# StractOrg/stract

Hardware: AMD Instinct MI355X
Metric: HyperBall traversed edges/sec (GTEPS) (higher is better)
Workload: dtype u8

## Files before the change

stract_amd/_lib.py:

```python
import ctypes
import os

os.environ.setdefault("OMP_WAIT_POLICY", "passive")

import numpy as np

_HERE = os.path.dirname(os.path.abspath(__file__))
LIB_PATH = os.environ.get("HB_LIB_PATH") or os.path.join(_HERE, "lib", "libhyperball.so")
LIB_EXP_PATH = os.environ.get("HB_LIB_PATH") or os.path.join(_HERE, "lib", "libhyperball_exp.so")

HB_OK = 0
HB_ERR_INVALID, HB_ERR_NO_DEVICE, HB_ERR_HIP, HB_ERR_NOMEM, HB_ERR_RCCL, HB_ERR_LIMIT, HB_ERR_IO = -1, -2, -3, -4, -5, -6, -7
HB_STORE_F64, HB_STORE_U64 = 0, 1
HB_COLL_U8, HB_COLL_U32, HB_COLL_U64, HB_COLL_F64 = 0, 1, 2, 3
HB_COLL_MAX, HB_COLL_SUM = 0, 1
HB_SKIPPED_REL_MASK = 0x6FED00

HB_FLAG_NO_FRONTIER = 0x01
HB_FLAG_NO_REORDER = 0x02
HB_FLAG_UNFUSED = 0x04
HB_FLAG_PASS_STATS = 0x08
HB_FLAG_NO_XCD_MAP = 0x20
HB_FLAG_NO_RCCL = 0x40
HB_FLAG_RCCL_SELF = 0x80
HB_FLAG_NO_SPARSE = 0x100
HB_FLAG_DEST_PARTITION = 0x200
HB_FLAG_HOST_INGEST = 0x400
HB_FLAG_HOST_PLAN = 0x800
HB_FLAG_CHANGED_ONLY = 0x1000
HB_FLAG_REFERENCE_TAIL = 0x2000
HB_FLAG_NO_INIT_PASS = 0x4000
HB_FLAG_ALL_RELS = 0x8000
HB_SAMPLE_MAX_LEVELS = 16

HB_X_TILE_EPILOGUE = 0x100
HB_X_SEED_3LAUNCH = 0x800
HB_X_NO_EDGE_OVERLAP = 0x1000
HB_X_BITMAP_SLOTWISE = 0x2000
HB_X_NO_STAGED_RESULTS = 0x4000
HB_X_SNAPSHOT_EVERY_PASS = 0x8000
HB_X_SHORT_FINAL_LIST = 0x10000
HB_X_ONE_SNAPSHOT = 0x20000
HB_X_NO_TAIL_PIPELINE = 0x100000
HB_X_TAIL_KERNEL = 0x200000
HB_X_TAIL_KERNEL_ANY = 0x400000
HB_X_FULL_INIT = 0x800000
HB_X_WIRE_64B = 0x1000000
HB_X_SCATTER_TRANSPOSE = 0x2000000
HB_X_SWEEP_ROUNDS = 0x4000000
HB_X_GENERIC_LEVEL1 = 0x8000000
HB_X_PROBE_NO_SIZE = 0x10000000

U128 = np.dtype([("lo", "<u8"), ("hi", "<u8")])
EDGE = np.dtype([("from", U128), ("to", U128), ("rel_flags", "<u8")])
assert U128.itemsize == 16 and EDGE.itemsize == 40


class HbOptions(ctypes.Structure):
    _fields_ = [
        ("struct_size", ctypes.c_uint32),
        ("device", ctypes.c_int32),
        ("flags", ctypes.c_uint32),
        ("chunk", ctypes.c_uint32),
        ("max_passes", ctypes.c_uint32),
        ("rank", ctypes.c_int32),
        ("world_size", ctypes.c_int32),
        ("rccl_id", ctypes.c_uint8 * 128),
        ("tune", ctypes.c_uint32 * 8),
    ]


class HbStats(ctypes.Structure):
    _fields_ = [
        ("n", ctypes.c_uint64),
        ("m_input", ctypes.c_uint64),
        ("m_unique", ctypes.c_uint64),
        ("m_eff", ctypes.c_uint64),
        ("passes", ctypes.c_uint64),
        ("results", ctypes.c_uint64),
        ("ms_ingest", ctypes.c_double),
        ("ms_plan", ctypes.c_double),
        ("ms_h2d", ctypes.c_double),
        ("ms_loop", ctypes.c_double),
        ("ms_loop_gpu", ctypes.c_double),
        ("ms_collective", ctypes.c_double),
        ("ms_d2h", ctypes.c_double),
        ("work_rows", ctypes.c_uint64),
        ("virtual_rows", ctypes.c_uint64),
        ("device_bytes", ctypes.c_uint64),
        ("virtual_edges", ctypes.c_uint64),
        ("levels", ctypes.c_uint64),
        ("level1_edges", ctypes.c_uint64),
        ("level1_rows", ctypes.c_uint64),
        ("direct_edges", ctypes.c_uint64),
        ("rows_with_in_edges", ctypes.c_uint64),
# ... 971 lines not shown
```

stract_amd/csrc/hb_api.hip:

```cpp
#include "hb_guard_alloc.h"
#include "hb_pool.h"
#include <hip/hip_runtime.h>
#include <rccl/rccl.h>

#include <algorithm>
#include <cmath>
#include <cstdio>
#include <cstring>
#include <string>
#include <thread>
#include <vector>

#include "hb_internal.h"
#include "hb_experiments.h"
#include "hb_kernels.hip.h"
#include "hb_walk.hip.h"
#include "hb_sample.hip.h"
#include "hb_bfs.hip.h"
#include "hb_betweenness.hip.h"
#include "hb_similarity.hip.h"
#include "hb_nearest_seed.hip.h"
#ifdef HB_EXPERIMENTS
#include "hb_experiments.hip.h"
#endif
// ... 61 lines not shown
};
}

struct GraphDeviceState {
    uint64_t *d_row_ptr = nullptr;
    uint32_t *d_src = nullptr;
    uint16_t *d_src_jp = nullptr;
    bool level0_all_real = false;
    uint32_t *d_virt_rows = nullptr;
    uint16_t *d_self_jp = nullptr;
    uint4 *d_regs[2] = {nullptr, nullptr};
    uint4 *d_part = nullptr;
    uint32_t *d_bits[2] = {nullptr, nullptr};
    uint32_t *d_kdirty = nullptr;
    double *d_ksum = nullptr, *d_kerr = nullptr;
    uint64_t *d_size = nullptr;
    uint64_t *d_idlow = nullptr;
    uint32_t *d_dev_of = nullptr;
    uint32_t *d_sid_of = nullptr;
    uint32_t *d_outdeg = nullptr;
    unsigned long long *d_counters = nullptr;
    double *d_raw = nullptr, *d_bias = nullptr;
    uint8_t *d_lc = nullptr;
    uint64_t *d_out_ptr = nullptr;
    uint32_t *d_out_rows = nullptr;
    uint32_t *d_touch = nullptr;
    uint32_t *d_seeds = nullptr, *d_heavy = nullptr;
    unsigned int *d_sparse_counts = nullptr;
    bool sparse_ok = false;
    uint4 *d_pack = nullptr;
    uint32_t *d_wpop = nullptr;
    uint64_t *d_wprefix = nullptr;
    uint32_t *d_lbits = nullptr, *d_lbits_all = nullptr, *d_ubits = nullptr;
    bool ubits_valid = false;
    unsigned long long *d_rank_cnt = nullptr;
    uint32_t *d_tl_changed[2] = {nullptr, nullptr}, *d_tl_vchanged[2] = {nullptr, nullptr}, *d_tl_dirty[2] = {nullptr, nullptr};
    uint32_t *d_tl_work = nullptr, *d_tl_count = nullptr;
    bool tl_valid = false;
    uint64_t *d_tail_ptr = nullptr;
    uint32_t *d_tail_to = nullptr;
    uint64_t tail_count = 0;
    std::vector<uint64_t> tail_keys;
    std::vector<TailDoc> tail_open;
    bool tail_dirty = false;
    TailIndex *tail_index = nullptr;
    uint32_t *d_bloom = nullptr;
    unsigned long long *d_bloom_ones = nullptr;
    uint32_t *d_list = nullptr;
    double *d_out = nullptr;
    double *h_out = nullptr;
    uint64_t h_out_len = 0;
    uint64_t out_len = 0;
    uint32_t *d_cid_of = nullptr;
    std::vector<uint64_t> h_in_bits;
    struct ResultSync {
        bool on = false;
        bool valid = false;
        uint64_t changed_since = 0;
        uint32_t stages = 0;
        double *d_sent = nullptr;
        uint32_t *d_sid = nullptr;
        double *d_val = nullptr;
        unsigned long long *d_count = nullptr;
        unsigned long long *d_kept = nullptr;
        uint32_t *h_sid = nullptr;
        double *h_val = nullptr;
        unsigned long long *h_count = nullptr;
        uint64_t cap = 0;
    } rs;
    struct SampleState {
        DevPtr<uint16_t> d_hist;
        uint32_t levels = 0;
        DevPtr<unsigned long long> d_cnt;
        DevPtr<uint32_t> d_srcs;
        DevPtr<uint32_t> d_rows;
        DevPtr<double> d_w;
        std::vector<uint32_t> cand;
        bool cand_valid = false;
    } smp;
    struct DistanceState {
        bool ready = false;
        bool valid = false;
        bool extracted = false;
        uint8_t *d_dist = nullptr;
        uint32_t *d_vis = nullptr, *d_front = nullptr, *d_next = nullptr;
        uint32_t *d_heavy = nullptr;
        uint32_t heavy_cap = 0;
        unsigned int *d_heavy_cnt = nullptr;
        unsigned long long *d_cnt = nullptr;
        uint32_t *d_indeg = nullptr;
        bool indeg_valid = false;
        uint8_t *d_by_sid = nullptr;
        uint32_t *d_sel_sid = nullptr;
        uint8_t *d_sel_dist = nullptr;
        uint64_t *d_sel_cnt = nullptr;
        uint64_t words_total = 0;
        uint64_t reached = 0;
    } dst;
    struct BetweennessState {
        bool ready = false;
        bool valid = false;
        uint8_t *d_dist = nullptr;
        unsigned long long *d_sigma = nullptr;
        double *d_delta = nullptr;
        uint8_t *d_reached = nullptr;
        double *d_sum = nullptr;
// ... 1016 lines not shown
        const Plan &p = c->plan;
        double t0 = now_ms();
        if ((rc = ensure_initial_state(c))) return rc;
        if (linked(c) && p.n_pad) {
            HB_COLL(coll_all_gather(c, c->d_ksum + (uint64_t)c->opt.rank * c->slice_rows, c->d_ksum, c->slice_rows, ncclDouble, c->stream));
        }
        const double norm = (double)(p.n ? p.n - 1 : 0);
        unsigned long long *cnt = c->d_counters + (size_t)c->max_passes * hbk::kCounterWords;
        HB_HIP(hipMemsetAsync(cnt, 0, hbk::kCounterWords * sizeof(unsigned long long), c->stream));
        bool shipped = false;
        if (p.n && c->rs.on && c->rs.valid) {
            auto &rs = c->rs;
            HB_HIP(hipMemsetAsync(rs.d_count, 0, sizeof(unsigned long long), c->stream));
            const unsigned blocks = grid_blocks(c, (p.n_pad + 2047) / 2048, 8);
            hipLaunchKernelGGL(hbk::results_sync_kernel, dim3(blocks), dim3(256), 0, c->stream, (const double *)c->d_ksum, rs.d_sent,
                               (const uint32_t *)c->d_cid_of, p.n_pad, norm, 0, c->d_out, rs.d_sid, rs.d_val, (unsigned long long)rs.cap, rs.d_count, cnt);
            HB_HIP(hipGetLastError());
            HB_HIP(hipMemcpyAsync(rs.h_count, rs.d_count, sizeof(unsigned long long), hipMemcpyDeviceToHost, c->stream));
            HB_HIP(hipMemcpyAsync(c->h_counters, cnt, hbk::kCounterWords * sizeof(unsigned long long), hipMemcpyDeviceToHost, c->stream));
            HB_HIP(hipStreamSynchronize(c->stream));
            const uint64_t moved = *rs.h_count;
            if (moved <= rs.cap) {
                if (moved) {
                    HB_HIP(hipMemcpyAsync(rs.h_sid, rs.d_sid, moved * sizeof(uint32_t), hipMemcpyDeviceToHost, c->stream));
                    HB_HIP(hipMemcpyAsync(rs.h_val, rs.d_val, moved * sizeof(double), hipMemcpyDeviceToHost, c->stream));
                    HB_HIP(hipStreamSynchronize(c->stream));
                }
                HB_HIP(hipEventSynchronize(c->rs_copied));
                host_scatter_f64(c->h_out, rs.h_sid, rs.h_val, moved);
            } else {
                HB_HIP(hipStreamWaitEvent(c->stream, c->rs_copied, 0));
                HB_HIP(hipMemcpyAsync(c->h_out, c->d_out, c->out_len * sizeof(double), hipMemcpyDeviceToHost, c->stream));
                HB_HIP(hipStreamSynchronize(c->stream));
            }
            shipped = true;
        }
        if (p.n && !shipped) {
            if (c->rs.on) {
                const unsigned blocks = grid_blocks(c, (p.n_pad + 2047) / 2048, 8);
                hipLaunchKernelGGL(hbk::results_sync_kernel, dim3(blocks), dim3(256), 0, c->stream, (const double *)c->d_ksum, c->rs.d_sent,
                                   (const uint32_t *)c->d_cid_of, p.n_pad, norm, 1, c->d_out, (uint32_t *)nullptr, (double *)nullptr, 0ull, c->rs.d_count, cnt);
            } else {
                unsigned blocks = grid_blocks(c, (p.n + 255) / 256, 8);
                hipLaunchKernelGGL(hbk::finish_kernel, dim3(blocks), dim3(256), 0, c->stream, (const double *)c->d_ksum,
                                   (const uint32_t *)c->d_dev_of, p.n, norm, c->d_out, cnt);
            }
            HB_HIP(hipGetLastError());
            HB_HIP(hipMemcpyAsync(c->h_out, c->d_out, c->out_len * sizeof(double), hipMemcpyDeviceToHost, c->stream));
        }
        if (!shipped) {
            HB_HIP(hipMemcpyAsync(c->h_counters, cnt, hbk::kCounterWords * sizeof(unsigned long long), hipMemcpyDeviceToHost, c->stream));
            HB_HIP(hipStreamSynchronize(c->stream));
        }
        if (std::getenv("HB_TRACE_RESULTS"))
            std::fprintf(stderr, "[hb results] hb_finish: entered at %.3f ms, done at %.3f ms (host clock); %u snapshots, list %llu\n", t0, now_ms(), c->rs.stages,
                         shipped ? (unsigned long long)*c->rs.h_count : 0ull);
        c->stats.pipelined_passes = c->pipelined_passes;
        c->stats.tail_kernel_passes = c->tail_kernel_passes;
        c->stats.result_stages = c->rs.stages;
        c->stats.result_list = shipped ? *c->rs.h_count : 0;
        c->rs.valid = false;
        c->res_count = 0;
        for (int s = 0; s < hbk::kStripes; s++) c->res_count += c->h_counters[4 * s];
        c->stats.ms_d2h = now_ms() - t0;
        c->stats.results = c->res_count;
        c->stats.passes = c->t;
        if ((rc = resolve_pass_times(c))) return rc;
        double g = 0, coll = 0;
        for (auto &ps : c->pstats) { g += ps.ms_gpu; coll += ps.ms_collective; }
        c->stats.ms_loop_gpu = g;
        c->stats.ms_collective = coll;
        c->stats.wire_bytes = c->wire_bytes;
        c->run_open = false;
        c->image = Image::HyperBall;
        return HB_OK;
    });
}

int hb_run(hb_ctx *c, hb_stats *stats)
{
    return guarded(c, [&]() -> int {
        if (!c) return HB_ERR_INVALID;
        int rc = hb_begin(c);
        if (rc) return rc;
        double t0 = now_ms();
        int has = 1;
        const bool trace = std::getenv("HB_TRACE_RESULTS") != nullptr;
        while (has) {
            if (tail_kernel_ready(c)) {
                uint32_t ran = 0;
                if ((rc = tail_kernel_run(c, 64, &ran))) return rc;
                has = c->has_changes ? 1 : 0;
                if (ran) continue;
            }
            if (tail_pipeline_ready(c)) {
                if ((rc = tail_pipeline(c, &has))) return rc;
                continue;
            }
            if ((rc = hb_step(c, &has))) return rc;
            if (trace) std::fprintf(stderr, "[hb results] pass %llu returned at %.3f ms (host clock)\n", (unsigned long long)c->t - 1, now_ms());
        }
        c->stats.ms_loop = now_ms() - t0;
        if ((rc = hb_finish(c))) return rc;
        if (stats) *stats = c->stats;
        return HB_OK;
    });
// ... 147 lines not shown
```

stract_amd/csrc/hb_api_load.inc:

```
bool device_plan(const hb_ctx *c) { return !(c->opt.flags & HB_FLAG_HOST_PLAN); }
bool deferred_times(const hb_ctx *c);

int keep_owned(hb_ctx *c, DeviceCsr *csr)
{
    if (!dest_mode(c)) return HB_OK;
    const uint64_t world = (uint64_t)std::max(c->opt.world_size, 1), rank = (uint64_t)c->opt.rank, n = c->g.ids.size();
    if (c->g.row_ptr.size() == n + 1 && n) keep_owned_rows(&c->g, world, rank);
    if (csr && csr->d_row_ptr) {
        const std::string e = gpu_keep_owned_rows((void *)c->stream, csr, n, world, rank);
        if (!e.empty()) return fail(c, e.find("memory") != std::string::npos ? HB_ERR_NOMEM : HB_ERR_HIP, e);
    }
    return HB_OK;
}

__global__ __launch_bounds__(256) void idlow_kernel(const uint64_t *lo_by_sid, const uint32_t *order, uint64_t n_pad, uint64_t *idlow)
{
    const uint64_t d = (uint64_t)blockIdx.x * 256 + threadIdx.x;
    if (d >= n_pad) return;
    const uint32_t s = order[d];
    idlow[d] = s == kNone ? 0ull : lo_by_sid[s];
}

template <class T>
T *adopt(hb_ctx *c, DevPtr<T> &b, size_t bytes)
// ... 234 lines not shown
            HB_HIP(hipMemcpyAsync(c->d_src, p.src.data(), p.src.size() * sizeof(uint32_t), hipMemcpyHostToDevice, c->stream));
        if (p.n_pad)
            HB_HIP(hipMemcpyAsync(c->d_sid_of, p.order.data(), p.n_pad * sizeof(uint32_t), hipMemcpyHostToDevice, c->stream));
        std::vector<uint32_t> outdeg_dev(p.n_pad, 0);
        c->m_global = 0;
        for (uint64_t d = 0; d < p.n_pad; d++)
            if (p.order[d] != kNone) {
                outdeg_dev[d] = outdeg[p.order[d]];
                c->m_global += outdeg[p.order[d]];
            }
        if (p.n_pad)
            HB_HIP(hipMemcpyAsync(c->d_outdeg, outdeg_dev.data(), p.n_pad * sizeof(uint32_t), hipMemcpyHostToDevice, c->stream));
        if (n) HB_HIP(hipMemcpyAsync(c->d_dev_of, p.dev_of.data(), n * sizeof(uint32_t), hipMemcpyHostToDevice, c->stream));
        HB_HIP(hipStreamSynchronize(c->stream));
    } else {
        uint64_t ends[2] = {0, 0};
        HB_HIP(hipMemcpyAsync(&ends[0], c->d_row_ptr + p.n_pad, sizeof(uint64_t), hipMemcpyDeviceToHost, c->stream));
        HB_HIP(hipMemcpyAsync(&ends[1], c->d_row_ptr + rows_total, sizeof(uint64_t), hipMemcpyDeviceToHost, c->stream));
        HB_HIP(hipStreamSynchronize(c->stream));
        c->stats.virtual_edges = ends[1] - ends[0];
    }
    lap("tables / plan arrays");
    c->out_len = n;
    c->d_cid_of = c->d_sid_of;
    if (c->rs.on && n) {
        DevPtr<uint32_t> d_flags;
        DevPtr<uint64_t> d_cpos;
        DevPtr<unsigned long long> d_words;
        const uint64_t nw = (n + 63) / 64;
        HB_HIP(d_flags.alloc(n + 1));
        HB_HIP(d_cpos.alloc(n + 2));
        HB_HIP(d_words.alloc(nw));
        if ((rc = dev_alloc(c, &c->d_cid_of, p.n_pad))) return rc;
        HB_HIP(hipMemsetAsync(d_flags.get(), 0, (n + 1) * sizeof(uint32_t), c->stream));
        const unsigned blocks = grid_blocks(c, (p.n_pad + 255) / 256, 16);
        hipLaunchKernelGGL(hbk::in_flags_kernel, dim3(blocks), dim3(256), 0, c->stream, (const uint64_t *)c->d_row_ptr, (const uint32_t *)c->d_sid_of, p.n_pad, d_flags.get());
        HB_HIP(hipGetLastError());
        const std::string e = device_prefix((void *)c->stream, d_flags.get(), n, d_cpos.get());
        if (!e.empty()) return fail(c, HB_ERR_HIP, e);
        hipLaunchKernelGGL(hbk::cid_of_kernel, dim3(blocks), dim3(256), 0, c->stream, (const uint64_t *)c->d_row_ptr, (const uint32_t *)c->d_sid_of,
                           (const uint64_t *)d_cpos.get(), p.n_pad, c->d_cid_of);
        HB_HIP(hipGetLastError());
        hipLaunchKernelGGL(hbk::pack_flags_kernel, dim3(grid_blocks(c, (nw + 3) / 4, 16)), dim3(256), 0, c->stream,
                           (const uint32_t *)d_flags.get(), n, d_words.get());
        HB_HIP(hipGetLastError());
        uint64_t n_c = 0;
        c->h_in_bits.assign(nw, 0);
        HB_HIP(hipMemcpyAsync(&n_c, d_cpos.get() + n, sizeof(uint64_t), hipMemcpyDeviceToHost, c->stream));
        HB_HIP(hipMemcpyAsync(c->h_in_bits.data(), d_words.get(), nw * sizeof(uint64_t), hipMemcpyDeviceToHost, c->stream));
        HB_HIP(hipStreamSynchronize(c->stream));
        if (n_c != p.rows_with_in_edges)
            return fail(c, HB_ERR_INVALID, "result image: " + std::to_string(n_c) + " nodes with in-edges counted on the device, the plan says " + std::to_string(p.rows_with_in_edges));
        c->out_len = n_c;
        lap("compact result image (cid per row, host bitmap)");
    }
    if (n) {
        if (!d_lo) {
            uvec<uint64_t> lo(n);
            host_gather_id_lo(c->g.ids.data(), n, lo.data());
            HB_HIP(d_lo.alloc(n));
            HB_HIP(hipMemcpyAsync(d_lo.get(), lo.data(), n * sizeof(uint64_t), hipMemcpyHostToDevice, c->stream));
            HB_HIP(hipStreamSynchronize(c->stream));
        }
        hipLaunchKernelGGL(idlow_kernel, dim3((unsigned)((p.n_pad + 255) / 256)), dim3(256), 0, c->stream, (const uint64_t *)d_lo.get(),
                           (const uint32_t *)c->d_sid_of, p.n_pad, c->d_idlow);
        HB_HIP(hipGetLastError());
        HB_HIP(hipStreamSynchronize(c->stream));
    }
    lap("id_low");
    if (src_len && !(c->opt.flags & HB_FLAG_NO_INIT_PASS)) {
        if ((rc = dev_alloc(c, &c->d_src_jp, src_len + 4))) return rc;
        const unsigned blocks = grid_blocks(c, (src_len + 255) / 256, 16);
        if ((rc = dev_alloc(c, &c->d_self_jp, p.n_pad + 4))) return rc;
        hipLaunchKernelGGL(hbk::self_jp_kernel, dim3(grid_blocks(c, (p.n_pad + 255) / 256, 16)), dim3(256), 0, c->stream,
                           (const uint64_t *)c->d_idlow, (const uint32_t *)c->d_sid_of, p.n_pad, c->d_self_jp);
        HB_HIP(hipGetLastError());
        hipLaunchKernelGGL(hbk::src_jp_kernel, dim3(blocks), dim3(256), 0, c->stream, (const uint32_t *)c->d_src, src_len, (const uint16_t *)c->d_self_jp, p.n_pad,
                           c->d_src_jp);
        HB_HIP(hipGetLastError());
        if ((rc = dev_alloc(c, &c->d_virt_rows, c->bits_words + 4))) return rc;
        unsigned long long *d_l0 = c->d_counters + 8, h_l0 = ~0ull;
        HB_HIP(hipMemsetAsync(d_l0, 0, sizeof(unsigned long long), c->stream));
        const uint64_t l0_lo = p.level_begin.size() > 1 ? p.level_begin[0] : 0, l0_hi = p.level_begin.size() > 1 ? p.level_begin[1] : 0;
        hipLaunchKernelGGL(hbk::virt_rows_kernel, dim3(grid_blocks(c, (rows_total + 255) / 256, 16)), dim3(256), 0, c->stream,
                           (const uint64_t *)c->d_row_ptr, (const uint32_t *)c->d_src, rows_total, p.n_pad, c->d_virt_rows, l0_lo, l0_hi, d_l0);
        HB_HIP(hipGetLastError());
        HB_HIP(hipMemcpyAsync(&h_l0, d_l0, sizeof(h_l0), hipMemcpyDeviceToHost, c->stream));
        HB_HIP(hipStreamSynchronize(c->stream));
        c->level0_all_real = h_l0 == 0;
        HB_HIP(hipStreamSynchronize(c->stream));
    }
    lap("self_jp / src_jp");
    {
        unsigned long long *d_bad = c->d_counters;
        unsigned long long h_bad[4] = {0, 0, 0, 0};
        HB_HIP(hipMemsetAsync(d_bad, 0, sizeof(h_bad), c->stream));
        if (rows_total) {
            const unsigned blocks = grid_blocks(c, (rows_total * 4 + 255) / 256, 16);
            hipLaunchKernelGGL(hbk::validate_plan_kernel, dim3(blocks), dim3(256), 0, c->stream, (const uint64_t *)c->d_row_ptr, (const uint32_t *)c->d_src,
                               rows_total, p.n_pad, src_len, d_bad);
            HB_HIP(hipGetLastError());
        }
        HB_HIP(hipMemcpyAsync(h_bad, d_bad, sizeof(h_bad), hipMemcpyDeviceToHost, c->stream));
        HB_HIP(hipStreamSynchronize(c->stream));
        if (h_bad[0] | h_bad[1] | h_bad[2] | h_bad[3])
            return fail(c, HB_ERR_INVALID, "work layout failed its structural check: " + std::to_string(h_bad[0]) + " bad row pointers, " +
                                               std::to_string(h_bad[1]) + " source ids out of range, " + std::to_string(h_bad[2]) +
// ... 74 lines not shown
```

stract_amd/csrc/hb_api_pass.inc:

```
using PassKernel = void (*)(const hbk::PassParams);
using SweepKernel = void (*)(const hbk::SweepParams);

template <bool REAL, bool FUSED, bool STATS, bool INIT, bool EPI4>
PassKernel dense_by_unroll(int unroll)
{
    if constexpr (!INIT) {
        if (unroll == 1) return hbk::pass_kernel<REAL, FUSED, STATS, 1, INIT, EPI4>;
    }
    if (unroll == 2) return hbk::pass_kernel<REAL, FUSED, STATS, 2, INIT, EPI4>;
    return hbk::pass_kernel<REAL, FUSED, STATS, 4, INIT, EPI4>;
}
template <bool REAL, bool FUSED>
PassKernel dense_kernel_of(bool stats, int unroll, bool init, bool epi4)
{
    if (stats) return dense_by_unroll<REAL, FUSED, true, false, false>(unroll);
    if constexpr (REAL && FUSED) {
        if (epi4) return init ? dense_by_unroll<true, true, false, true, true>(unroll) : dense_by_unroll<true, true, false, false, true>(unroll);
    }
    return init ? dense_by_unroll<REAL, FUSED, false, true, false>(unroll) : dense_by_unroll<REAL, FUSED, false, false, false>(unroll);
}
PassKernel dense_kernel(bool real, bool fused, bool stats, int unroll, bool init, bool epi4)
{
    init = init && unroll != 1;
    if (real && fused) return dense_kernel_of<true, true>(stats, unroll, init, epi4);
// ... 348 lines not shown
        }
        if (!c->exact_counting && bloom_estimate_card(c->bloom_bits, ones) <= c->ref_threshold) c->exact_counting = true;
    }
    c->exact_valid = tracked;
    return HB_OK;
}

int upload_tail_index(hb_ctx *c)
{
    const Plan &p = c->plan;
    std::vector<uint64_t> ptr;
    std::vector<uint32_t> to;
    const std::string e = build_tail_csr(&c->tail_keys, p.n_pad, &ptr, &to);
    if (!e.empty()) return fail(c, HB_ERR_NOMEM, e);
    for (void *old : {(void *)c->d_tail_ptr, (void *)c->d_tail_to}) {
        if (!old) continue;
        for (size_t i = 0; i < c->allocs.size(); i++)
            if (c->allocs[i].p == old) {
                c->stats.device_bytes -= c->allocs[i].bytes;
                (void)hipFree(old);
                c->allocs.erase(c->allocs.begin() + (long)i);
                break;
            }
    }
    c->d_tail_ptr = nullptr;
    c->d_tail_to = nullptr;
    int rc;
    if ((rc = dev_alloc(c, &c->d_tail_ptr, p.n_pad + 1))) return rc;
    if ((rc = dev_alloc(c, &c->d_tail_to, to.size() + 1))) return rc;
    HB_HIP(hipMemcpyAsync(c->d_tail_ptr, ptr.data(), (p.n_pad + 1) * sizeof(uint64_t), hipMemcpyHostToDevice, c->stream));
    if (!to.empty()) HB_HIP(hipMemcpyAsync(c->d_tail_to, to.data(), to.size() * sizeof(uint32_t), hipMemcpyHostToDevice, c->stream));
    HB_HIP(hipStreamSynchronize(c->stream));
    c->tail_count = to.size();
    c->tail_dirty = false;
    return HB_OK;
}

using hbk::PassMode;
using hbk::kModeDense;
using hbk::kModeBitmap;
using hbk::kModeSweep;
bool below_dense_threshold(const hb_ctx *c, uint64_t active_edges)
{
    const uint32_t thr = c->opt.tune[2] ? c->opt.tune[2] : 50;
    return active_edges * 100ull < (uint64_t)thr * c->m_global;
}
PassMode pass_mode(const hb_ctx *c, uint64_t active_edges)
{
    if ((c->opt.flags & HB_FLAG_NO_FRONTIER) || !(below_dense_threshold(c, active_edges) || c->opt.tune[2] > 100)) return kModeDense;
    const uint64_t sparse_div = c->opt.tune[6] ? c->opt.tune[6] : 10;
    return c->sparse_ok && (active_edges * sparse_div < c->m_global || c->opt.tune[6] == 1) ? kModeSweep : kModeBitmap;
}

int results_stage(hb_ctx *c)
{
    const Plan &p = c->plan;
    auto &rs = c->rs;
    const double norm = (double)(p.n ? p.n - 1 : 0);
    hipLaunchKernelGGL(hbk::results_sync_kernel, dim3(grid_blocks(c, (p.n_pad + 2047) / 2048, 8)), dim3(256), 0, c->stream, (const double *)c->d_ksum, rs.d_sent, (const uint32_t *)c->d_cid_of,
                       p.n_pad, norm, rs.valid ? 0 : 1, c->d_out, (uint32_t *)nullptr, (double *)nullptr, 0ull, rs.d_count, rs.d_kept);
    HB_HIP(hipGetLastError());
    HB_HIP(hipEventRecord(c->rs_ready, c->stream));
    HB_HIP(hipStreamWaitEvent(c->rs_stream, c->rs_ready, 0));
    HB_HIP(hipMemcpyAsync(c->h_out, c->d_out, c->out_len * sizeof(double), hipMemcpyDeviceToHost, c->rs_stream));
    HB_HIP(hipEventRecord(c->rs_copied, c->rs_stream));
    if (std::getenv("HB_TRACE_RESULTS")) std::fprintf(stderr, "[hb results] snapshot %u queued after pass %llu at %.3f ms (host clock)\n", rs.stages + 1, (unsigned long long)c->t - 1, now_ms());
    rs.valid = true;
    rs.changed_since = 0;
    rs.stages++;
    return HB_OK;
}
int results_stage_policy(hb_ctx *c, uint64_t changed)
{
    auto &rs = c->rs;
    if (!rs.on || !c->has_changes) return HB_OK;
    rs.changed_since += changed;
    const bool forced = xbit(c, HB_X_SNAPSHOT_EVERY_PASS);
    bool go;
    if (!rs.valid) go = forced || below_dense_threshold(c, c->last_active);
    else go = (forced || rs.changed_since * 8 > c->plan.n) && !xbit(c, HB_X_ONE_SNAPSHOT) && hipEventQuery(c->rs_copied) == hipSuccess;
    (void)hipGetLastError();
    return go ? results_stage(c) : HB_OK;
}

hbk::SweepParams make_sweep_params(const hb_ctx *c, const hbk::PassParams &pp, unsigned slot, const unsigned long long *guard)
{
    hbk::SweepParams sp{};
    sp.p = pp;
    sp.out_ptr = c->d_out_ptr;
    sp.out_rows = c->d_out_rows;
    sp.touch = c->d_touch;
    sp.seeds = c->d_seeds;
    sp.heavy = c->d_heavy;
    sp.counts = c->d_sparse_counts + 2 * slot;
    sp.counts_next = c->d_sparse_counts + 2 * (slot ^ 1);
    sp.guard = guard;
    return sp;
}

void launch_sweep_seeding(hb_ctx *c, const hbk::SweepParams &sp, bool small)
{
    const unsigned sblocks = grid_blocks(c, sp.p.n_pad / 32 / 256, 4, 1);
    const unsigned wblocks = (unsigned)c->num_cu * 4;
    if (small) {
        hipLaunchKernelGGL(hbk::sweep_seed_small_kernel, dim3(sblocks), dim3(256), 0, c->stream, sp);
    } else {
        hipLaunchKernelGGL(hbk::sweep_collect_kernel, dim3(sblocks), dim3(256), 0, c->stream, sp);
        hipLaunchKernelGGL(hbk::sweep_expand_kernel, dim3(wblocks), dim3(256), 0, c->stream, sp);
        hipLaunchKernelGGL(hbk::sweep_expand_heavy_kernel, dim3(wblocks), dim3(256), 0, c->stream, sp);
    }
}

int sweep_pass(hb_ctx *c, const hbk::PassParams &pp, hipEvent_t *E)
{
    const Plan &p = c->plan;
    hbk::SweepParams sp = make_sweep_params(c, pp, (unsigned)(c->t & 1), c->spec_guard);
    launch_sweep_seeding(c, sp, c->last_changed <= 4096 && !xbit(c, HB_X_SEED_3LAUNCH));
    HB_HIP(hipEventRecord(E[kEvLevel1], c->stream));
    const bool by_rounds = xbit(c, HB_X_SWEEP_ROUNDS);
// ... 422 lines not shown
        if ((rc = results_stage_policy(c, c->last_changed))) return rc;
        if (!c->has_changes) break;
        if (!ahead) {
            if (has_changes) *has_changes = 1;
            return HB_OK;
        }
        if (c->last_changed > 4096 || c->cur_mode != 2 || tail_kernel_ready(c)) {
            if ((rc = tail_complete(c))) return rc;
            if ((rc = results_stage_policy(c, c->last_changed))) return rc;
            break;
        }
    }
    if (has_changes) *has_changes = c->has_changes ? 1 : 0;
    return HB_OK;
}

int warm_kernels(hb_ctx *c)
{
    if (!c->plan.n_pad || (c->opt.flags & HB_FLAG_PASS_STATS)) return HB_OK;
    hbk::PassParams pp = make_params(c);
    pp.row_lo = pp.row_hi = 0;
    pp.xcd_map = 0;
    pp.n_pad = 0;
    pp.counters = c->d_counters + (size_t)c->max_passes * hbk::kCounterWords;
    hipStream_t s = c->stream;
    const dim3 one(1), blk(256);
    const bool fused = !unfused(c), epi4 = !xbit(c, HB_X_TILE_EPILOGUE), compact = !xbit(c, HB_X_BITMAP_SLOTWISE);
    const int hub_unroll = pass_unroll(c, false), node_unroll = pass_unroll(c, true);
    auto warm = [&](PassKernel k) { hipLaunchKernelGGL(k, one, blk, 0, s, pp); };
    warm(dense_kernel(false, false, false, hub_unroll, false, false));
    warm(dense_kernel(true, fused, false, node_unroll, false, epi4));
    if (fused && pass0_streams_initial_registers(c)) {
        warm(dense_kernel(false, false, false, hub_unroll, true, false));
        warm(hbk::init_level1_kernel);
        warm(dense_kernel(true, true, false, node_unroll, true, epi4));
    }
    warm(bitmap_kernel(false, false, false, compact));
    warm(bitmap_kernel(true, fused, false, compact));
    if (!fused) warm(hbk::epilogue_kernel);
    if (c->sparse_ok) {
        const hbk::SweepParams sp = make_sweep_params(c, pp, 0, nullptr);
        HB_HIP(hipMemsetAsync(c->d_sparse_counts, 0, 64 * sizeof(unsigned int), s));
        hipLaunchKernelGGL(hbk::sweep_collect_kernel, one, blk, 0, s, sp);
        hipLaunchKernelGGL(hbk::sweep_expand_kernel, one, blk, 0, s, sp);
        hipLaunchKernelGGL(hbk::sweep_expand_heavy_kernel, one, blk, 0, s, sp);
        hipLaunchKernelGGL(hbk::sweep_seed_small_kernel, one, blk, 0, s, sp);
        const bool by_rounds = xbit(c, HB_X_SWEEP_ROUNDS);
        hipLaunchKernelGGL(sweep_rows_kernel_for(false, by_rounds), one, blk, 0, s, sp);
        hipLaunchKernelGGL(sweep_rows_kernel_for(true, by_rounds), one, blk, 0, s, sp);
    }
    if (c->rs.on) {
        hipLaunchKernelGGL(hbk::results_sync_kernel, one, blk, 0, s, (const double *)c->d_ksum, c->rs.d_sent, (const uint32_t *)c->d_cid_of, (uint64_t)0, 1.0, 0,
                           c->d_out, (uint32_t *)nullptr, (double *)nullptr, 0ull, c->rs.d_count, pp.counters);
    }
    hipLaunchKernelGGL(hbk::finish_kernel, one, blk, 0, s, (const double *)c->d_ksum, (const uint32_t *)c->d_dev_of, (uint64_t)0, 1.0, c->d_out, pp.counters);
    HB_HIP(hipGetLastError());
    return HB_OK;
}
```

stract_amd/csrc/hb_aux.hip.h:

```cpp
#pragma once

namespace hbk {

__global__ __launch_bounds__(256) void validate_plan_kernel(const uint64_t *row_ptr, const uint32_t *src, uint64_t rows_total, uint64_t n_pad,
                                                            uint64_t src_len, unsigned long long *bad)
{
    const uint64_t t = (uint64_t)blockIdx.x * 256 + threadIdx.x;
    const uint64_t nq = (uint64_t)gridDim.x * 64;
    const int q = threadIdx.x & 3;
    unsigned b0 = 0, b1 = 0, b2 = 0, b3 = 0;
    for (uint64_t row = t >> 2; row < rows_total; row += nq) {
        const uint64_t b = row_ptr[row], e = row_ptr[row + 1];
        if (b > e || e > src_len) {
            b0 += (q == 0);
            continue;
        }
        if (row + 1 == rows_total && e != src_len) b0 += (q == 0);
        const bool first_virtual = b < e && src[b] >= n_pad;
        for (uint64_t k = b + q; k < e; k += 4) {
            const uint32_t s = src[k];
            if (s >= rows_total) b1++;
            else {
                if ((s >= n_pad) != first_virtual) b2++;
                if (s >= n_pad && (row < n_pad ? false : s >= row)) b3++;
// ... 225 lines not shown
        const uint32_t from = rd[u * 16 + w];
        const uint64_t e = tail_ptr[u + 1];
        for (uint64_t j = tail_ptr[u] + k; j < e; j += 4) {
            uint32_t *dst = &wr[(uint64_t)tail_to[j] * 16 + w];
            uint32_t old = __hip_atomic_load(dst, __ATOMIC_RELAXED, __HIP_MEMORY_SCOPE_AGENT);
            for (;;) {
                const uint32_t nw = bytes_max(old, from);
                if (nw == old) break;
                const uint32_t prev = atomicCAS(dst, old, nw);
                if (prev == old) break;
                old = prev;
            }
        }
    }
}

__device__ __forceinline__ double normalized_centrality(double s, double norm, bool &kept)
{
    double v = -1.0;
    kept = s > 0.0;
    if (kept) {
        v = s / norm;
        if (!(fabs(v) <= 1.7976931348623157e308)) v = 0.0;
    }
    return v;
}
__global__ __launch_bounds__(256) void finish_kernel(const double *ksum, const uint32_t *dev_of, uint64_t n,
                                                     double norm, double *out, unsigned long long *count)
{
    unsigned long long kept = 0;
    for (uint64_t sid = (uint64_t)blockIdx.x * 256 + threadIdx.x; sid < n; sid += (uint64_t)gridDim.x * 256) {
        bool k;
        out[sid] = normalized_centrality(ksum[dev_of[sid]], norm, k);
        kept += k;
    }
#pragma unroll
    for (int off = 32; off > 0; off >>= 1) kept += __shfl_down(kept, off);
    const unsigned long long v[4] = {kept, 0, 0, 0};
    block_add_counters(count, v, 0x1u);
}

__global__ __launch_bounds__(256) void in_flags_kernel(const uint64_t *row_ptr, const uint32_t *sid_of, uint64_t n_pad, uint32_t *flags)
{
    for (uint64_t row = (uint64_t)blockIdx.x * 256 + threadIdx.x; row < n_pad; row += (uint64_t)gridDim.x * 256) {
        const uint32_t sd = sid_of[row];
        if (sd != kNone) flags[sd] = row_ptr[row + 1] > row_ptr[row] ? 1u : 0u;
    }
}
__global__ __launch_bounds__(256) void cid_of_kernel(const uint64_t *row_ptr, const uint32_t *sid_of, const uint64_t *cpos, uint64_t n_pad, uint32_t *cid_of)
{
    for (uint64_t row = (uint64_t)blockIdx.x * 256 + threadIdx.x; row < n_pad; row += (uint64_t)gridDim.x * 256) {
        const uint32_t sd = sid_of[row];
        cid_of[row] = (sd != kNone && row_ptr[row + 1] > row_ptr[row]) ? (uint32_t)cpos[sd] : kNone;
    }
}
__global__ __launch_bounds__(256) void pack_flags_kernel(const uint32_t *flags, uint64_t n, unsigned long long *words)
{
    const uint64_t nw = (n + 63) >> 6;
    for (uint64_t w = (uint64_t)blockIdx.x * 4 + (threadIdx.x >> 6); w < nw; w += (uint64_t)gridDim.x * 4) {
        const uint64_t i = (w << 6) + (threadIdx.x & 63);
        const unsigned long long m = __ballot(i < n && flags[i] != 0u);
        if ((threadIdx.x & 63) == 0) words[w] = m;
    }
}

constexpr int kSyncPerThread = 8;
__global__ __launch_bounds__(256) void results_sync_kernel(const double *ksum, double *sent, const uint32_t *sid_of, uint64_t n_pad, double norm,
                                                           int all, double *out, uint32_t *list_sid, double *list_val, unsigned long long cap,
                                                           unsigned long long *counts, unsigned long long *count)
{
    __shared__ uint32_t s_wave[4];
    __shared__ unsigned long long s_base;
    const int lane = threadIdx.x & 63, wave = threadIdx.x >> 6;
    unsigned long long kept = 0;
    const uint64_t span = 256ull * kSyncPerThread;
    for (uint64_t base = (uint64_t)blockIdx.x * span; base < n_pad; base += (uint64_t)gridDim.x * span) {
        uint32_t mask = 0, sid[kSyncPerThread];
        double val[kSyncPerThread];
#pragma unroll
        for (int j = 0; j < kSyncPerThread; j++) {
            const uint64_t row = base + (uint64_t)j * 256 + threadIdx.x;
            sid[j] = kNone;
            val[j] = 0.0;
            if (row < n_pad) {
                const uint32_t sd = sid_of[row];
                if (sd != kNone) {
                    const double s = ksum[row];
                    bool k;
                    const double v = normalized_centrality(s, norm, k);
                    kept += k;
                    if (all || __double_as_longlong(s) != __double_as_longlong(sent[row])) {
                        sent[row] = s;
                        out[sd] = v;
                        mask |= 1u << j;
                        sid[j] = sd;
                        val[j] = v;
                    }
                }
            }
        }
        if (list_sid) {
            const uint32_t mine = __popc(mask);
            uint32_t incl = mine;
#pragma unroll
            for (int off = 1; off < 64; off <<= 1) {
                const uint32_t a = __shfl_up(incl, off);
                if (lane >= off) incl += a;
            }
            if (lane == 63) s_wave[wave] = incl;
            __syncthreads();
            if (threadIdx.x == 0) {
                const uint32_t tot = s_wave[0] + s_wave[1] + s_wave[2] + s_wave[3];
                s_base = tot ? atomicAdd(counts, (unsigned long long)tot) : 0ull;
            }
            __syncthreads();
            unsigned long long pos = s_base + (incl - mine);
            for (int w = 0; w < wave; w++) pos += s_wave[w];
#pragma unroll
            for (int j = 0; j < kSyncPerThread; j++) {
                if ((mask >> j) & 1u) {
                    if (pos < cap) {
                        list_sid[pos] = sid[j];
                        list_val[pos] = val[j];
                    }
                    pos++;
                }
            }
            __syncthreads();
        }
    }
#pragma unroll
    for (int off = 32; off > 0; off >>= 1) kept += __shfl_down(kept, off);
    const unsigned long long v[4] = {kept, 0, 0, 0};
    block_add_counters(count, v, 0x1u);
}

__device__ __forceinline__ uint64_t hash_mix64(uint64_t x)
{
    x ^= x >> 33;
    x *= 0xff51afd7ed558ccdull;
    x ^= x >> 33;
    x *= 0xc4ceb9fe1a85ec53ull;
    x ^= x >> 33;
    return x;
}
__global__ __launch_bounds__(256) void state_hash_kernel(const uint4 *regs, const double *ksum, const double *kerr,
                                                         const uint32_t *dev_of, uint64_t n, unsigned long long *out)
{
    unsigned long long hr = 0, hk = 0;
    for (uint64_t sid = (uint64_t)blockIdx.x * 256 + threadIdx.x; sid < n; sid += (uint64_t)gridDim.x * 256) {
        const uint64_t row = dev_of[sid];
        uint64_t r = sid * 0x9E3779B97F4A7C15ull + 1ull;
#pragma unroll
        for (int k = 0; k < 4; k++) {
            const uint4 v = regs[row * 4 + k];
            r = hash_mix64(r ^ (((uint64_t)v.y << 32) | v.x));
            r = hash_mix64(r ^ (((uint64_t)v.w << 32) | v.z));
        }
        hr += r;
        const uint64_t a = (uint64_t)__double_as_longlong(ksum[row]), b = (uint64_t)__double_as_longlong(kerr[row]);
        hk += hash_mix64(hash_mix64((sid + 0x632BE59BD9B4E019ull) ^ a) ^ b);
    }
#pragma unroll
    for (int off = 32; off > 0; off >>= 1) {
        hr += __shfl_down(hr, off);
        hk += __shfl_down(hk, off);
    }
    const unsigned long long v[4] = {hr, hk, 0, 0};
    block_add_counters(out, v, 0x3u);
}

__global__ __launch_bounds__(256) void gather_rows_kernel(const uint4 *regs, const uint32_t *dev_of, uint64_t n,
                                                          uint4 *out)
{
    const uint64_t t = (uint64_t)blockIdx.x * 256 + threadIdx.x;
    const uint64_t sid = t >> 2;
    if (sid >= n) return;
    out[t] = regs[(uint64_t)dev_of[sid] * 4 + (t & 3)];
}

}
```

stract_amd/csrc/hb_experiments.h:

```cpp
#pragma once
#include <stdint.h>

#define HB_TUNE1_UNROLL 0xFFu
#ifdef HB_EXPERIMENTS
#define HB_XBITS(tune1) ((uint32_t)(tune1) & ~HB_TUNE1_UNROLL)
#else
#define HB_XBITS(tune1) 0u
#endif

enum hb_xbit : uint32_t {
    HB_X_TILE_EPILOGUE = 0x100u,
    HB_X_SEED_3LAUNCH = 0x800u,
    HB_X_NO_EDGE_OVERLAP = 0x1000u,
    HB_X_BITMAP_SLOTWISE = 0x2000u,
    HB_X_NO_STAGED_RESULTS = 0x4000u,
    HB_X_SNAPSHOT_EVERY_PASS = 0x8000u,
    HB_X_SHORT_FINAL_LIST = 0x10000u,
    HB_X_ONE_SNAPSHOT = 0x20000u,
    HB_X_NO_TAIL_PIPELINE = 0x100000u,
    HB_X_TAIL_KERNEL = 0x200000u,
    HB_X_TAIL_KERNEL_ANY = 0x400000u,
    HB_X_FULL_INIT = 0x800000u,
    HB_X_WIRE_64B = 0x1000000u,
    HB_X_SCATTER_TRANSPOSE = 0x2000000u,
    HB_X_SWEEP_ROUNDS = 0x4000000u,
    HB_X_GENERIC_LEVEL1 = 0x8000000u,
    HB_X_PROBE_NO_SIZE = 0x10000000u,
};
```

Measured before the change: 111.9.

## Stream first result snapshot in compact-id slices overlapping device-to-host copies

Builds an inverse map from compact result id to device row at load time. The first full result snapshot during sweep-mode passes is then produced in eight slices, each walking compact ids directly and followed by its own async device-to-host copy on the results stream. This lets the copy of earlier slices overlap with computing later ones and avoids scanning all padded rows. It costs an extra device array, an extra load-time kernel plus sync, and more launches and event records per snapshot.

New measurement: 110.6. 0.988x the previous value.

```diff
diff --git a/stract_amd/_lib.py b/stract_amd/_lib.py
--- a/stract_amd/_lib.py
+++ b/stract_amd/_lib.py
@@ -41,6 +41,7 @@
 HB_X_SNAPSHOT_EVERY_PASS = 0x8000
 HB_X_SHORT_FINAL_LIST = 0x10000
 HB_X_ONE_SNAPSHOT = 0x20000
+HB_X_SNAPSHOT_DEVICE_ORDER = 0x40000
 HB_X_NO_TAIL_PIPELINE = 0x100000
 HB_X_TAIL_KERNEL = 0x200000
 HB_X_TAIL_KERNEL_ANY = 0x400000
diff --git a/stract_amd/csrc/hb_api.hip b/stract_amd/csrc/hb_api.hip
--- a/stract_amd/csrc/hb_api.hip
+++ b/stract_amd/csrc/hb_api.hip
@@ -137,6 +137,7 @@
     uint64_t h_out_len = 0;
     uint64_t out_len = 0;
     uint32_t *d_cid_of = nullptr;
+    uint32_t *d_row_of_cid = nullptr;
     std::vector<uint64_t> h_in_bits;
     struct ResultSync {
         bool on = false;
@@ -1259,6 +1260,17 @@
             HB_HIP(hipMemcpyAsync(c->h_counters, cnt, hbk::kCounterWords * sizeof(unsigned long long), hipMemcpyDeviceToHost, c->stream));
             HB_HIP(hipStreamSynchronize(c->stream));
         }
+#ifdef HB_DEBUG_BOUNDS
+        if (p.n && c->out_len) {
+            std::vector<double> check(c->out_len);
+            HB_HIP(hipStreamSynchronize(c->stream));
+            if (c->rs_stream) HB_HIP(hipStreamSynchronize(c->rs_stream));
+            HB_HIP(hipMemcpy(check.data(), c->d_out, c->out_len * sizeof(double), hipMemcpyDeviceToHost));
+            for (uint64_t i = 0; i < c->out_len; i++)
+                if (std::memcmp(&check[i], &c->h_out[i], sizeof(double)) != 0)
+                    return fail(c, HB_ERR_INVALID, "HB_DEBUG_BOUNDS: h_out[" + std::to_string(i) + "] differs from d_out after hb_finish");
+        }
+#endif
         if (std::getenv("HB_TRACE_RESULTS"))
             std::fprintf(stderr, "[hb results] hb_finish: entered at %.3f ms, done at %.3f ms (host clock); %u snapshots, list %llu\n", t0, now_ms(), c->rs.stages,
                          shipped ? (unsigned long long)*c->rs.h_count : 0ull);
diff --git a/stract_amd/csrc/hb_api_load.inc b/stract_amd/csrc/hb_api_load.inc
--- a/stract_amd/csrc/hb_api_load.inc
+++ b/stract_amd/csrc/hb_api_load.inc
@@ -310,7 +310,26 @@
         if (n_c != p.rows_with_in_edges)
             return fail(c, HB_ERR_INVALID, "result image: " + std::to_string(n_c) + " nodes with in-edges counted on the device, the plan says " + std::to_string(p.rows_with_in_edges));
         c->out_len = n_c;
-        lap("compact result image (cid per row, host bitmap)");
+        if ((rc = dev_alloc(c, &c->d_row_of_cid, std::max<uint64_t>(n_c, 1)))) return rc;
+        hipLaunchKernelGGL(hbk::row_of_cid_kernel, dim3(blocks), dim3(256), 0, c->stream, (const uint32_t *)c->d_cid_of, p.n_pad, n_c, c->d_row_of_cid);
+        HB_HIP(hipGetLastError());
+        HB_HIP(hipStreamSynchronize(c->stream));
+#ifdef HB_DEBUG_BOUNDS
+        {
+            std::vector<uint32_t> h_cid(p.n_pad), h_row(n_c);
+            if (p.n_pad) HB_HIP(hipMemcpy(h_cid.data(), c->d_cid_of, p.n_pad * sizeof(uint32_t), hipMemcpyDeviceToHost));
+            if (n_c) HB_HIP(hipMemcpy(h_row.data(), c->d_row_of_cid, n_c * sizeof(uint32_t), hipMemcpyDeviceToHost));
+            uint64_t in_image = 0;
+            for (uint64_t row = 0; row < p.n_pad; row++) {
+                if (h_cid[row] == kNone) continue;
+                in_image++;
+                if (h_cid[row] >= n_c || h_row[h_cid[row]] != row)
+                    return fail(c, HB_ERR_INVALID, "HB_DEBUG_BOUNDS: row_of_cid is not the inverse of cid_of at device row " + std::to_string(row));
+            }
+            if (in_image != n_c) return fail(c, HB_ERR_INVALID, "HB_DEBUG_BOUNDS: " + std::to_string(in_image) + " rows in the compact image of " + std::to_string(n_c) + " entries");
+        }
+#endif
+        lap("compact result image (cid per row and its inverse, host bitmap)");
     }
     if (n) {
         if (!d_lo) {
diff --git a/stract_amd/csrc/hb_api_pass.inc b/stract_amd/csrc/hb_api_pass.inc
--- a/stract_amd/csrc/hb_api_pass.inc
+++ b/stract_amd/csrc/hb_api_pass.inc
@@ -424,19 +424,48 @@
     return c->sparse_ok && (active_edges * sparse_div < c->m_global || c->opt.tune[6] == 1) ? kModeSweep : kModeBitmap;
 }
 
-int results_stage(hb_ctx *c)
+constexpr int kResultSlices = 8;
+int results_stage_slices(hb_ctx *c)
 {
     const Plan &p = c->plan;
     auto &rs = c->rs;
     const double norm = (double)(p.n ? p.n - 1 : 0);
-    hipLaunchKernelGGL(hbk::results_sync_kernel, dim3(grid_blocks(c, (p.n_pad + 2047) / 2048, 8)), dim3(256), 0, c->stream, (const double *)c->d_ksum, rs.d_sent, (const uint32_t *)c->d_cid_of,
-                       p.n_pad, norm, rs.valid ? 0 : 1, c->d_out, (uint32_t *)nullptr, (double *)nullptr, 0ull, rs.d_count, rs.d_kept);
-    HB_HIP(hipGetLastError());
-    HB_HIP(hipEventRecord(c->rs_ready, c->stream));
-    HB_HIP(hipStreamWaitEvent(c->rs_stream, c->rs_ready, 0));
-    HB_HIP(hipMemcpyAsync(c->h_out, c->d_out, c->out_len * sizeof(double), hipMemcpyDeviceToHost, c->rs_stream));
+    const uint64_t len = c->out_len, per = ((len + kResultSlices - 1) / kResultSlices + 15) & ~15ull;
+    const uint64_t span = 256ull * hbk::kSlicePerThread;
+    for (int k = 0; k < kResultSlices; k++) {
+        const uint64_t lo = std::min(len, (uint64_t)k * per), hi = std::min(len, lo + per);
+        if (lo >= hi) continue;
+        hipLaunchKernelGGL(hbk::results_slice_kernel, dim3(grid_blocks(c, (hi - lo + span - 1) / span, 8)), dim3(256), 0, c->stream, (const double *)c->d_ksum, rs.d_sent,
+                           (const uint32_t *)c->d_row_of_cid, norm, c->d_out, lo, hi);
+        HB_HIP(hipGetLastError());
+        HB_HIP(hipEventRecord(c->rs_ready, c->stream));
+        HB_HIP(hipStreamWaitEvent(c->rs_stream, c->rs_ready, 0));
+        HB_HIP(hipMemcpyAsync(c->h_out + lo, c->d_out + lo, (hi - lo) * sizeof(double), hipMemcpyDeviceToHost, c->rs_stream));
+    }
     HB_HIP(hipEventRecord(c->rs_copied, c->rs_stream));
-    if (std::getenv("HB_TRACE_RESULTS")) std::fprintf(stderr, "[hb results] snapshot %u queued after pass %llu at %.3f ms (host clock)\n", rs.stages + 1, (unsigned long long)c->t - 1, now_ms());
+    return HB_OK;
+}
+int results_stage(hb_ctx *c)
+{
+    const Plan &p = c->plan;
+    auto &rs = c->rs;
+    const bool slices = !rs.valid && c->d_row_of_cid && pass_mode(c, c->last_active) == kModeSweep && !xbit(c, HB_X_SNAPSHOT_DEVICE_ORDER);
+    if (slices) {
+        const int rc = results_stage_slices(c);
+        if (rc) return rc;
+    } else {
+        const double norm = (double)(p.n ? p.n - 1 : 0);
+        hipLaunchKernelGGL(hbk::results_sync_kernel, dim3(grid_blocks(c, (p.n_pad + 2047) / 2048, 8)), dim3(256), 0, c->stream, (const double *)c->d_ksum, rs.d_sent, (const uint32_t *)c->d_cid_of,
+                           p.n_pad, norm, rs.valid ? 0 : 1, c->d_out, (uint32_t *)nullptr, (double *)nullptr, 0ull, rs.d_count, rs.d_kept);
+        HB_HIP(hipGetLastError());
+        HB_HIP(hipEventRecord(c->rs_ready, c->stream));
+        HB_HIP(hipStreamWaitEvent(c->rs_stream, c->rs_ready, 0));
+        HB_HIP(hipMemcpyAsync(c->h_out, c->d_out, c->out_len * sizeof(double), hipMemcpyDeviceToHost, c->rs_stream));
+        HB_HIP(hipEventRecord(c->rs_copied, c->rs_stream));
+    }
+    if (std::getenv("HB_TRACE_RESULTS"))
+        std::fprintf(stderr, "[hb results] snapshot %u (%s) queued after pass %llu at %.3f ms (host clock)\n", rs.stages + 1, slices ? "slices" : "device order",
+                     (unsigned long long)c->t - 1, now_ms());
     rs.valid = true;
     rs.changed_since = 0;
     rs.stages++;
@@ -965,6 +994,8 @@
     if (c->rs.on) {
         hipLaunchKernelGGL(hbk::results_sync_kernel, one, blk, 0, s, (const double *)c->d_ksum, c->rs.d_sent, (const uint32_t *)c->d_cid_of, (uint64_t)0, 1.0, 0,
                            c->d_out, (uint32_t *)nullptr, (double *)nullptr, 0ull, c->rs.d_count, pp.counters);
+        if (c->d_row_of_cid)
+            hipLaunchKernelGGL(hbk::results_slice_kernel, one, blk, 0, s, (const double *)c->d_ksum, c->rs.d_sent, (const uint32_t *)c->d_row_of_cid, 1.0, c->d_out, (uint64_t)0, (uint64_t)0);
     }
     hipLaunchKernelGGL(hbk::finish_kernel, one, blk, 0, s, (const double *)c->d_ksum, (const uint32_t *)c->d_dev_of, (uint64_t)0, 1.0, c->d_out, pp.counters);
     HB_HIP(hipGetLastError());
diff --git a/stract_amd/csrc/hb_aux.hip.h b/stract_amd/csrc/hb_aux.hip.h
--- a/stract_amd/csrc/hb_aux.hip.h
+++ b/stract_amd/csrc/hb_aux.hip.h
@@ -301,6 +301,13 @@
     for (uint64_t row = (uint64_t)blockIdx.x * 256 + threadIdx.x; row < n_pad; row += (uint64_t)gridDim.x * 256) {
         const uint32_t sd = sid_of[row];
         cid_of[row] = (sd != kNone && row_ptr[row + 1] > row_ptr[row]) ? (uint32_t)cpos[sd] : kNone;
+    }
+}
+__global__ __launch_bounds__(256) void row_of_cid_kernel(const uint32_t *cid_of, uint64_t n_pad, uint64_t out_len, uint32_t *row_of_cid)
+{
+    for (uint64_t row = (uint64_t)blockIdx.x * 256 + threadIdx.x; row < n_pad; row += (uint64_t)gridDim.x * 256) {
+        const uint32_t cid = cid_of[row];
+        if (cid != kNone && cid < out_len) row_of_cid[cid] = (uint32_t)row;
     }
 }
 __global__ __launch_bounds__(256) void pack_flags_kernel(const uint32_t *flags, uint64_t n, unsigned long long *words)
@@ -384,6 +391,31 @@
     block_add_counters(count, v, 0x1u);
 }
 
+constexpr int kSlicePerThread = 4;
+__global__ __launch_bounds__(256) void results_slice_kernel(const double *ksum, double *sent, const uint32_t *row_of_cid, double norm, double *out,
+                                                            uint64_t cid_lo, uint64_t cid_hi)
+{
+    const uint64_t span = 256ull * kSlicePerThread;
+    for (uint64_t base = cid_lo + (uint64_t)blockIdx.x * span; base < cid_hi; base += (uint64_t)gridDim.x * span) {
+        uint32_t row[kSlicePerThread];
+        double s[kSlicePerThread];
+#pragma unroll
+        for (int j = 0; j < kSlicePerThread; j++) {
+            const uint64_t cid = base + (uint64_t)j * 256 + threadIdx.x;
+            row[j] = cid < cid_hi ? row_of_cid[cid] : kNone;
+        }
+#pragma unroll
+        for (int j = 0; j < kSlicePerThread; j++) s[j] = row[j] != kNone ? ksum[row[j]] : 0.0;
+#pragma unroll
+        for (int j = 0; j < kSlicePerThread; j++) {
+            if (row[j] == kNone) continue;
+            bool k;
+            sent[row[j]] = s[j];
+            out[base + (uint64_t)j * 256 + threadIdx.x] = normalized_centrality(s[j], norm, k);
+        }
+    }
+}
+
 __device__ __forceinline__ uint64_t hash_mix64(uint64_t x)
 {
     x ^= x >> 33;
diff --git a/stract_amd/csrc/hb_experiments.h b/stract_amd/csrc/hb_experiments.h
--- a/stract_amd/csrc/hb_experiments.h
+++ b/stract_amd/csrc/hb_experiments.h
@@ -17,6 +17,7 @@
     HB_X_SNAPSHOT_EVERY_PASS = 0x8000u,
     HB_X_SHORT_FINAL_LIST = 0x10000u,
     HB_X_ONE_SNAPSHOT = 0x20000u,
+    HB_X_SNAPSHOT_DEVICE_ORDER = 0x40000u,
     HB_X_NO_TAIL_PIPELINE = 0x100000u,
     HB_X_TAIL_KERNEL = 0x200000u,
     HB_X_TAIL_KERNEL_ANY = 0x400000u,
```
